# fateshelled/onnx_image_processing

Hardware: AMD Instinct MI355X
Metric: image-pairs/sec (640x480, K=512) (higher is better)
Workload: dtype f32; 1 GPU; Shi-Tomasi(3) + NMS(r=5)/top-k + sparse BAD(512, hard) + Sinkhorn(20, eps 0.05) + MNN(100, 0.1), 640x480 gray pairs, K=512 (BASELINE configs[1]); height=480, width=640, max_keypoints=512, parallelism=pair-sharded x1, input=float32 frames resident in HBM

## Files before the change

### onnx_image_processing_amd/csrc/hooks.h

```cpp
#pragma once

#ifdef MI_DEBUG_HOOKS
#include <atomic>
struct MiHooks {
  std::atomic<int> corner_impl{0};
  std::atomic<int> corner_rows{4};
  std::atomic<int> corner_rows_u8_default{1};
  std::atomic<int> sinkhorn_log_partials{0};
  std::atomic<int> sinkhorn_split{2};
  std::atomic<int> sinkhorn_persist{1};
  std::atomic<int> sinkhorn_stamps{0};
  std::atomic<int> topk_select{1};
  std::atomic<int> sinkhorn_schedule{-1};
  std::atomic<int> akaze_impl{0};
  std::atomic<int> bad_oriented_impl{0};
  std::atomic<int> cost_impl{0};
  std::atomic<int> sinkhorn_mix{1};
  std::atomic<int> sinkhorn_pair_waves{1};
  std::atomic<int> mnn_pair_waves{1};
  std::atomic<int> sinkhorn_exp_rows{1};
  std::atomic<int> mnn_one_pass{1};
  std::atomic<int> nms_impl{0};
  std::atomic<int> topk_split{-1};
  std::atomic<unsigned long long *> corner_clk{nullptr};
  std::atomic<unsigned long long *> topk_prof{nullptr};
};
extern MiHooks mi_hooks;
#define MI_HOOK(field, product_value) (mi_hooks.field.load(std::memory_order_relaxed))
#else
#define MI_HOOK(field, product_value) (product_value)
#endif
```

### onnx_image_processing_amd/csrc/hooks.hip

```cpp
#ifndef MI_DEBUG_HOOKS
#error "hooks.hip belongs to the debug library only (-DMI_DEBUG_HOOKS)"
#endif
#include "common.h"
#include "hooks.h"

#include "../../include/mi355x_match_debug.h"

MiHooks mi_hooks;

int mi_bad_plan_passes_host(const uint32_t *pair_geom_host, int num_pairs, int *canonical, int *scheduled);
int mi_sinkhorn_dots_form_host(int batch, int n, int m, int flags, int blocks_per_cu, int cus);

MI_API int mi_debug_clock_probe(void *buffer) {
  mi_hooks.corner_clk = reinterpret_cast<unsigned long long *>(buffer);
  return MI_OK;
}

MI_API int mi_debug_topk_stamps(void *buffer) {
  mi_hooks.topk_prof = reinterpret_cast<unsigned long long *>(buffer);
  return MI_OK;
}

MI_API int mi_debug_set(int key, int value) {
  if (key == 0) {
    mi_hooks.corner_impl = 0; mi_hooks.corner_rows = 4; mi_hooks.corner_rows_u8_default = 1;
    mi_hooks.sinkhorn_log_partials = 0; mi_hooks.sinkhorn_split = 2; mi_hooks.sinkhorn_persist = 1;
    mi_hooks.sinkhorn_stamps = 0; mi_hooks.topk_select = 1; mi_hooks.topk_split = -1; mi_hooks.sinkhorn_schedule = -1;
    mi_hooks.akaze_impl = 0;
    mi_hooks.bad_oriented_impl = 0;
    mi_hooks.cost_impl = 0;
    mi_hooks.sinkhorn_mix = 1;
    mi_hooks.sinkhorn_pair_waves = 1;
    mi_hooks.mnn_pair_waves = 1;
    mi_hooks.mnn_one_pass = 1;
    mi_hooks.sinkhorn_exp_rows = 1;
    mi_hooks.nms_impl = 0;
    mi_hooks.corner_clk = nullptr; mi_hooks.topk_prof = nullptr;
    return MI_OK;
  }
  if (key == 1) { mi_hooks.corner_impl = value; return MI_OK; }
  if (key == 2 && (value == 4 || value == 5 || value == 8)) { mi_hooks.corner_rows = value; mi_hooks.corner_rows_u8_default = 0; return MI_OK; }
  if (key == 4) { mi_hooks.sinkhorn_log_partials = value; return MI_OK; }
  if (key == 6) { mi_hooks.sinkhorn_split = value; return MI_OK; }
  if (key == 7) { mi_hooks.sinkhorn_persist = value; return MI_OK; }
  if (key == 8) { mi_hooks.sinkhorn_stamps = value; return MI_OK; }
  if (key == 9) { mi_hooks.topk_select = value; return MI_OK; }
  if (key == 10) { mi_hooks.topk_split = value; return MI_OK; }
  if (key == 12 && (value == 0 || value == 1)) { mi_hooks.akaze_impl = value; return MI_OK; }
  if (key == 13 && (value == 0 || value == 1)) { mi_hooks.bad_oriented_impl = value; return MI_OK; }
  if (key == 14 && (value == 0 || value == 1)) { mi_hooks.cost_impl = value; return MI_OK; }
  if (key == 15 && (value == 0 || value == 1)) { mi_hooks.sinkhorn_mix = value; return MI_OK; }
  if (key == 16 && (value == 0 || value == 1)) { mi_hooks.sinkhorn_pair_waves = value; return MI_OK; }
  if (key == 17 && (value == 0 || value == 1)) { mi_hooks.mnn_pair_waves = value; return MI_OK; }
  if (key == 19 && (value == 0 || value == 1)) { mi_hooks.mnn_one_pass = value; return MI_OK; }
  if (key == 18 && (value == 0 || value == 1)) { mi_hooks.sinkhorn_exp_rows = value; return MI_OK; }
  if (key == 20 && (value == 0 || value == 1)) { mi_hooks.nms_impl = value; return MI_OK; }
  if (key == 11 && value >= -1 && value <= 2) { mi_hooks.sinkhorn_schedule = value; return MI_OK; }
  return MI_E_PARAM;
}

MI_API int mi_debug_bad_plan_passes(const uint32_t *pair_geom_host, int num_pairs, int *canonical, int *scheduled) {
  return mi_bad_plan_passes_host(pair_geom_host, num_pairs, canonical, scheduled);
}

#include "sk_tuner.h"
MI_API int mi_debug_tuner_script(int n_ops, const int *op, const int *arg, const double *val, int *out) {
  if (n_ops < 0 || (n_ops > 0 && (!op || !arg || !val || !out))) return MI_E_NULL;
  mi::TunerLogic t;
  int last_entry = -1, last_slot = -1;
  for (int i = 0; i < n_ops; ++i) {
    mi::TunerShape s;
    s.batch = arg[i]; s.n = 512; s.m = 512; s.iterations = 20;
    switch (op[i]) {
      case 0: {
        const int sched = t.begin(s, &last_entry, &last_slot);
        out[i] = sched | ((last_slot & 0xff) << 8) | ((last_entry & 0xff) << 16);
        break;
      }
      case 1: t.finish(arg[i] >> 8, arg[i] & 0xff, val[i]); out[i] = 0; break;
      case 2: t.abandon(arg[i] >> 8, arg[i] & 0xff); out[i] = 0; break;
      case 3: out[i] = t.current(s); break;
      case 4: out[i] = t.for_capture(s); break;
      case 5: out[i] = t.set(arg[i]) ? 0 : -1; break;
      default: return MI_E_PARAM;
    }
  }
  return MI_OK;
}

MI_API int mi_debug_sinkhorn_dots_form(int batch, int n, int m, int flags, int blocks_per_cu, int cus) {
  return mi_sinkhorn_dots_form_host(batch, n, m, flags, blocks_per_cu, cus);
}

#include "akaze_math.h"
namespace {
__global__ __launch_bounds__(256) void akaze_math_check_kernel(int which, float kappa, uint32_t lo_bits, uint32_t hi_bits,
                                                               unsigned long long *mismatches, uint32_t *first_bad) {
  const float rk = 1.0f / kappa;
  unsigned long long bad = 0;
  for (unsigned long long b = (unsigned long long)lo_bits + blockIdx.x * 256ull + threadIdx.x; b < hi_bits;
       b += (unsigned long long)gridDim.x * 256ull) {
    const float x = __uint_as_float((uint32_t)b);
    float got, want;
    if (which == 0) { got = ak_sqrt(x); want = sqrtf(x); }
    else if (which == 1) { got = ak_div_by(x, kappa, rk); want = x / kappa; }
    else if (which == 2) { got = ak_rcp(x); want = 1.0f / x; }
    else if (which == 3) { got = ak_div(x, kappa); want = x / kappa; }
    else if (which == 4) { got = ak_sqrt_fp<1>(x); want = sqrtf(x); }
    else { got = ak_sqrt_fp<2>(x); want = sqrtf(x); }
    if (__float_as_uint(got) != __float_as_uint(want)) {
      ++bad;
      atomicMin(first_bad, (uint32_t)b);
    }
  }
  if (bad) atomicAdd(mismatches, bad);
}
}

MI_API int mi_debug_akaze_math_check(int which, float kappa, uint32_t lo_bits, uint32_t hi_bits, void *mismatches_u64,
                                     void *first_bad_u32, mi_stream_t stream) {
  MI_ENTER();
  if (!mismatches_u64 || !first_bad_u32) return MI_E_NULL;
  if (which < 0 || which > 5 || !(kappa > 0.0f) || lo_bits >= hi_bits) return MI_E_PARAM;
  hipLaunchKernelGGL(akaze_math_check_kernel, dim3(4096), dim3(256), 0, (hipStream_t)stream, which, kappa, lo_bits, hi_bits,
                     reinterpret_cast<unsigned long long *>(mismatches_u64), reinterpret_cast<uint32_t *>(first_bad_u32));
  return mi_launch_status();
}
```

### onnx_image_processing_amd/csrc/topk.hip

```cpp
#include "common.h"

#include "hooks.h"

namespace {

constexpr int TK_THREADS = 1024;
constexpr int TK_WAVES = TK_THREADS / 64;
constexpr int TK_MAX = 4096;
constexpr int TK_SEGS = 1024;

__device__ __forceinline__ void bitonic_sort_desc(uint64_t *keys, int npad, int t) {
  for (int size = 2; size <= npad; size <<= 1) {
    for (int stride = size >> 1; stride > 0; stride >>= 1) {
      for (int i = t; i < (npad >> 1); i += TK_THREADS) {
        const int pos = 2 * i - (i & (stride - 1));
        const int par = pos + stride;
        const bool desc = ((pos & size) == 0);
        const uint64_t a = keys[pos], b = keys[par];
        if ((a < b) == desc) {
          keys[pos] = b;
          keys[par] = a;
        }
      }
      __syncthreads();
    }
  }
}

template <int SIZE, int STRIDE>
__device__ __forceinline__ void bitonic_stage_4096(uint64_t (&r)[4], uint64_t *keys, uint64_t *keys2, int t, int &flip) {
  if constexpr (STRIDE < 4) {
#pragma unroll
    for (int j = 0; j < 4; ++j) {
      if ((j ^ STRIDE) > j) {
        const bool desc = (((t * 4 + j) & SIZE) == 0);
        const uint64_t a = r[j], b = r[j ^ STRIDE];
        const bool sw = (a < b) == desc;
        r[j] = sw ? b : a;
        r[j ^ STRIDE] = sw ? a : b;
      }
    }
  } else {
    uint64_t other[4];
    if constexpr (STRIDE < 256) {
#pragma unroll
      for (int j = 0; j < 4; ++j) other[j] = __shfl_xor(r[j], STRIDE >> 2, 64);
    } else {
      uint64_t *buf = flip ? keys2 : keys;
      flip ^= 1;
#pragma unroll
      for (int j = 0; j < 4; ++j) buf[t * 4 + j] = r[j];
      __syncthreads();
      const int pt = t ^ (STRIDE >> 2);
#pragma unroll
      for (int j = 0; j < 4; ++j) other[j] = buf[pt * 4 + j];
    }
    const bool lower = (t & (STRIDE >> 2)) == 0;
#pragma unroll
    for (int j = 0; j < 4; ++j) {
      const bool desc = (((t * 4 + j) & SIZE) == 0);
      const bool gt = r[j] > other[j];
      const uint64_t mx = gt ? r[j] : other[j], mn = gt ? other[j] : r[j];
      r[j] = (lower == desc) ? mx : mn;
    }
  }
}

template <int SIZE, int STRIDE>
__device__ __forceinline__ void bitonic_merge_4096(uint64_t (&r)[4], uint64_t *keys, uint64_t *keys2, int t, int &flip) {
  if constexpr (STRIDE >= 1) {
    bitonic_stage_4096<SIZE, STRIDE>(r, keys, keys2, t, flip);
    bitonic_merge_4096<SIZE, STRIDE / 2>(r, keys, keys2, t, flip);
  }
}

template <int SIZE>
__device__ __forceinline__ void bitonic_levels_4096(uint64_t (&r)[4], uint64_t *keys, uint64_t *keys2, int t, int &flip) {
  if constexpr (SIZE <= TK_MAX) {
    bitonic_merge_4096<SIZE, SIZE / 2>(r, keys, keys2, t, flip);
    bitonic_levels_4096<SIZE * 2>(r, keys, keys2, t, flip);
  }
}

__device__ __forceinline__ void bitonic_sort_desc_4096(uint64_t *keys, uint64_t *keys2, int t) {
  uint64_t r[4];
#pragma unroll
  for (int j = 0; j < 4; ++j) r[j] = keys[t * 4 + j];
  int flip = 0;
  bitonic_levels_4096<2>(r, keys, keys2, t, flip);
  __syncthreads();
#pragma unroll
  for (int j = 0; j < 4; ++j) keys[t * 4 + j] = r[j];
  __syncthreads();
}

constexpr int TK_BIG_MAX = 32768;

template <bool BIG>
__global__ __launch_bounds__(TK_THREADS) void topk_kernel(const uint64_t *__restrict__ cand,
                                                          const uint32_t *__restrict__ count, int segments,
                                                          uint32_t seg_cap, int w, int k, MiSets kpt_sets,
                                                          float *__restrict__ kscores, int select_mode,
                                                          unsigned long long *prof) {
#define TK_STAMP(i) do { if (prof && blockIdx.x == 0 && threadIdx.x == 0) prof[i] = wall_clock64(); } while (0)
  TK_STAMP(0);
  __shared__ uint64_t raw[BIG ? TK_BIG_MAX / 2 : 2 * TK_MAX];
  uint64_t *const keys = raw;
  uint64_t *const keys2 = raw + TK_MAX;
  uint32_t *const scores = reinterpret_cast<uint32_t *>(raw);
  __shared__ uint32_t seg_cnt[TK_SEGS], seg_base[TK_SEGS];
  __shared__ uint32_t hist[256];
  __shared__ uint32_t wsum[TK_WAVES];
  __shared__ uint64_t s_prefix;
  __shared__ uint32_t s_krem, s_fill, s_done;

  const int t = threadIdx.x, lane = t & 63, wave = t >> 6;
  const int img = blockIdx.x;
  const uint64_t *list = cand + (size_t)img * segments * seg_cap;
  const uint32_t *cnt = count + (size_t)img * segments;

  const bool slots = segments <= TK_SEGS;
  uint32_t part = 0;
  if (t == 0) s_fill = 0u;
  __syncthreads();
  for (int s = t; s < segments; s += TK_THREADS) {
    const uint32_t c = min(cnt[s], seg_cap);
    part += c;
    if (slots) {
      seg_cnt[s] = c;
      seg_base[s] = c ? atomicAdd(&s_fill, c) : 0u;
    }
  }
#pragma unroll
  for (int o = 32; o > 0; o >>= 1) part += __shfl_xor(part, o, 64);
  if (lane == 0) wsum[wave] = part;
  __syncthreads();
  uint32_t n = 0;
#pragma unroll
  for (int q = 0; q < TK_WAVES; ++q) n += wsum[q];
  int nsel;
  TK_STAMP(1);

  bool in_lds = false;
  if (BIG && slots && n > (uint32_t)TK_MAX && n <= (uint32_t)TK_BIG_MAX && k <= TK_MAX) {
    for (int s0 = wave * 8; s0 < segments; s0 += TK_WAVES * 8) {
      uint64_t v[8];
      uint32_t c[8], base[8];
#pragma unroll
      for (int q = 0; q < 8; ++q) {
        const int sg = s0 + q;
        c[q] = sg < segments ? seg_cnt[sg] : 0u;
        base[q] = sg < segments ? seg_base[sg] : 0u;
        v[q] = 0ull;
        if ((uint32_t)lane < c[q]) v[q] = list[(size_t)sg * seg_cap + lane];
      }
#pragma unroll
      for (int q = 0; q < 8; ++q) {
        if ((uint32_t)lane < c[q]) scores[base[q] + lane] = (uint32_t)(v[q] >> 32);
        for (uint32_t i = 64 + lane; i < c[q]; i += 64) scores[base[q] + i] = (uint32_t)(list[(size_t)(s0 + q) * seg_cap + i] >> 32);
      }
    }
    if (t == 0) { s_prefix = 0ull; s_krem = (uint32_t)k; s_done = 0u; }
    __syncthreads();
    uint32_t mask32 = 0u;
    for (int shift = 24; shift >= 0; shift -= 8) {
      if (t < 256) hist[t] = 0u;
      __syncthreads();
      const uint32_t prefix = (uint32_t)s_prefix;
      for (uint32_t i0 = 0; i0 < n; i0 += TK_THREADS) {
        const uint32_t i = i0 + t;
        const uint32_t sc = i < n ? scores[i] : 0u;
        const bool act = i < n && ((sc & mask32) == prefix);
        const uint32_t digit = (sc >> shift) & 255u;
        const unsigned long long am = __ballot(act);
        if (am) {
          const int leader = __ffsll((long long)am) - 1;
          const uint32_t d0 = __shfl(digit, leader, 64);
          const unsigned long long same = __ballot(act && digit == d0);
          if (lane == leader) atomicAdd(&hist[d0], (uint32_t)__popcll(same));
          if (act && digit != d0) atomicAdd(&hist[digit], 1u);
        }
      }
      __syncthreads();
      if (t < 64) {
        const uint32_t krem = s_krem;
        uint32_t c[4], tot = 0;
#pragma unroll
        for (int q = 0; q < 4; ++q) { c[q] = hist[255 - 4 * t - q]; tot += c[q]; }
        uint32_t incl = tot;
#pragma unroll
        for (int o = 1; o < 64; o <<= 1) {
          const uint32_t up = __shfl_up(incl, o, 64);
          if (t >= o) incl += up;
        }
        uint32_t above = incl - tot;
        if (above < krem && krem <= incl) {
#pragma unroll
          for (int q = 0; q < 4; ++q) {
            if (krem <= above + c[q]) {
              s_prefix = (uint64_t)(prefix | ((uint32_t)(255 - 4 * t - q) << shift));
              s_krem = krem - above;
              s_fill = c[q];
              if (krem - above == c[q]) s_done = 1u;
              break;
            }
            above += c[q];
          }
        }
      }
      mask32 |= (0xFFu << shift);
      __syncthreads();
      if (s_done) break;
    }
    const uint32_t floor32 = (uint32_t)s_prefix;
    const uint32_t n2 = ((uint32_t)k - s_krem) + s_fill;
    __syncthreads();
    if (n2 <= (uint32_t)TK_MAX) {
      if (t == 0) s_fill = 0u;
      __syncthreads();
      for (int s0 = wave * 8; s0 < segments; s0 += TK_WAVES * 8) {
        uint64_t v[8];
        uint32_t c[8];
#pragma unroll
        for (int q = 0; q < 8; ++q) {
          const int sg = s0 + q;
          c[q] = sg < segments ? seg_cnt[sg] : 0u;
          v[q] = 0ull;
          if ((uint32_t)lane < c[q]) v[q] = list[(size_t)sg * seg_cap + lane];
        }
#pragma unroll
        for (int q = 0; q < 8; ++q) {
          if ((uint32_t)lane < c[q] && (uint32_t)(v[q] >> 32) >= floor32) keys[atomicAdd(&s_fill, 1u)] = v[q];
          for (uint32_t i = 64 + lane; i < c[q]; i += 64) {
            const uint64_t key = list[(size_t)(s0 + q) * seg_cap + i];
            if ((uint32_t)(key >> 32) >= floor32) keys[atomicAdd(&s_fill, 1u)] = key;
          }
        }
      }
      __syncthreads();
      n = s_fill;
      in_lds = true;
    }
    __syncthreads();
  }

  if (in_lds || (n <= (uint32_t)TK_MAX && slots)) {
    for (int s0 = wave * 4; !in_lds && s0 < segments; s0 += TK_WAVES * 4) {
      uint64_t v[4];
      uint32_t c[4], base[4];
#pragma unroll
      for (int q = 0; q < 4; ++q) {
        const int sg = s0 + q;
        c[q] = sg < segments ? seg_cnt[sg] : 0u;
        base[q] = sg < segments ? seg_base[sg] : 0u;
        v[q] = 0ull;
        if ((uint32_t)lane < c[q]) v[q] = list[(size_t)sg * seg_cap + lane];
      }
#pragma unroll
      for (int q = 0; q < 4; ++q) {
        if ((uint32_t)lane < c[q]) keys[base[q] + lane] = v[q];
        for (uint32_t i = 64 + lane; i < c[q]; i += 64) keys[base[q] + i] = list[(size_t)(s0 + q) * seg_cap + i];
      }
    }
    int npad = 2;
    while (npad < (int)n) npad <<= 1;
    __syncthreads();
    TK_STAMP(2);
    if ((select_mode || in_lds) && n >= (uint32_t)k && 4 * k <= TK_MAX && (n > (uint32_t)k || in_lds)) {
      uint64_t r[4];
#pragma unroll
      for (int q = 0; q < 4; ++q) r[q] = (uint32_t)(t + q * TK_THREADS) < n ? keys[t + q * TK_THREADS] : 0ull;
      if (t == 0) { s_prefix = 0ull; s_krem = (uint32_t)k; s_fill = 0u; s_done = 0u; }
      uint64_t mask = 0ull;
      for (int shift = n == (uint32_t)k ? -8 : 56; shift >= 0; shift -= 8) {
        if (t < 256) hist[t] = 0u;
        __syncthreads();
        const uint64_t prefix = s_prefix;
#pragma unroll
        for (int q = 0; q < 4; ++q) {
          const bool act = r[q] != 0ull && ((r[q] & mask) == prefix);
          const uint32_t digit = (uint32_t)(r[q] >> shift) & 255u;
          const unsigned long long am = __ballot(act);
          if (am) {
            const int leader = __ffsll((long long)am) - 1;
            const uint32_t d0 = __shfl(digit, leader, 64);
            const unsigned long long same = __ballot(act && digit == d0);
            if (lane == leader) atomicAdd(&hist[d0], (uint32_t)__popcll(same));
            if (act && digit != d0) atomicAdd(&hist[digit], 1u);
          }
        }
        __syncthreads();
        if (t < 64) {
          const uint32_t krem = s_krem;
          uint32_t c[4], tot = 0;
#pragma unroll
          for (int q = 0; q < 4; ++q) { c[q] = hist[255 - 4 * t - q]; tot += c[q]; }
          uint32_t incl = tot;
#pragma unroll
          for (int o = 1; o < 64; o <<= 1) {
            const uint32_t up = __shfl_up(incl, o, 64);
            if (t >= o) incl += up;
          }
          uint32_t above = incl - tot;
          if (above < krem && krem <= incl) {
#pragma unroll
            for (int q = 0; q < 4; ++q) {
              if (krem <= above + c[q]) {
                s_prefix = prefix | ((uint64_t)(255 - 4 * t - q) << shift);
                s_krem = krem - above;
                if (krem - above == c[q]) s_done = 1u;
                break;
              }
              above += c[q];
            }
          }
        }
        mask |= (0xFFull << shift);
        __syncthreads();
        if (s_done) break;
      }
      if (n == (uint32_t)k) __syncthreads();
      const uint64_t kth = s_prefix;
      TK_STAMP(3);
#pragma unroll
      for (int q = 0; q < 4; ++q)
        if (r[q] != 0ull && r[q] >= kth) {
          const uint32_t slot = atomicAdd(&s_fill, 1u);
          if (slot < (uint32_t)TK_MAX) keys2[slot] = r[q];
        }
      __syncthreads();
      nsel = (int)(s_fill < (uint32_t)k ? s_fill : (uint32_t)k);
      int kpad = 2;
      while (kpad < k) kpad <<= 1;
      for (int i = nsel + t; i < kpad; i += TK_THREADS) keys2[i] = 0ull;
      __syncthreads();
      TK_STAMP(4);
      if (kpad >= 128 && kpad <= TK_THREADS) {
        const int tpk = TK_THREADS / kpad, slice = kpad / tpk;
        const int ki = t & (kpad - 1), part = t / kpad;
        if (t < kpad) seg_cnt[t] = 0u;
        const uint64_t mine = keys2[ki];
        uint32_t above = 0;
        if (mine != 0ull) {
          const ulonglong2 *lst = reinterpret_cast<const ulonglong2 *>(keys2 + part * slice);
#pragma unroll 8
          for (int j = 0; j < slice / 2; ++j) {
            const ulonglong2 two = lst[j];
            above += (two.x > mine ? 1u : 0u) + (two.y > mine ? 1u : 0u);
          }
        }
        __syncthreads();
        if (mine != 0ull && above) atomicAdd(&seg_cnt[ki], above);
        __syncthreads();
        if (part == 0 && mine != 0ull) keys[seg_cnt[ki]] = mine;
        __syncthreads();
      } else {
        bitonic_sort_desc(keys2, kpad, t);
        for (int i = t; i < nsel; i += TK_THREADS) keys[i] = keys2[i];
        __syncthreads();
      }
    } else {
    for (int i = (int)n + t; i < npad; i += TK_THREADS) keys[i] = 0ull;
    __syncthreads();
    if (npad == TK_MAX) bitonic_sort_desc_4096(keys, keys2, t);
    else bitonic_sort_desc(keys, npad, t);
    nsel = (int)n < k ? (int)n : k;
    }
  } else if (n <= (uint32_t)TK_MAX) {
    for (int s = wave; s < segments; s += TK_WAVES) {
      const uint32_t c = min(cnt[s], seg_cap);
      if (c == 0u) continue;
      uint32_t base = 0;
      if (lane == 0) base = atomicAdd(&s_fill, c);
      base = __shfl(base, 0, 64);
      const uint64_t *seg = list + (size_t)s * seg_cap;
      for (uint32_t i = lane; i < c; i += 64) keys[base + i] = seg[i];
    }
    int npad = 2;
    while (npad < (int)n) npad <<= 1;
    __syncthreads();
    for (int i = (int)n + t; i < npad; i += TK_THREADS) keys[i] = 0ull;
    __syncthreads();
    if (npad == TK_MAX) bitonic_sort_desc_4096(keys, keys2, t);
    else bitonic_sort_desc(keys, npad, t);
    nsel = (int)n < k ? (int)n : k;
  } else {
    if (t == 0) { s_prefix = 0ull; s_krem = (uint32_t)k; s_fill = 0u; s_done = 0u; }
    uint64_t mask = 0ull;
    for (int shift = 56; shift >= 0; shift -= 8) {
      if (t < 256) hist[t] = 0u;
      __syncthreads();
      const uint64_t prefix = s_prefix;
      for (int s = wave; s < segments; s += TK_WAVES) {
        const uint32_t c = min(cnt[s], seg_cap);
        const uint64_t *seg = list + (size_t)s * seg_cap;
        for (uint32_t base = 0; base < c; base += 64) {
          const uint32_t i = base + lane;
          bool act = false;
          uint32_t digit = 0;
          if (i < c) {
            const uint64_t key = seg[i];
            act = ((key & mask) == prefix);
            digit = (uint32_t)(key >> shift) & 255u;
          }
          const unsigned long long am = __ballot(act);
          if (am) {
            const int leader = __ffsll((long long)am) - 1;
            const uint32_t d0 = __shfl(digit, leader, 64);
            const unsigned long long same = __ballot(act && digit == d0);
            if (lane == leader) atomicAdd(&hist[d0], (uint32_t)__popcll(same));
            if (act && digit != d0) atomicAdd(&hist[digit], 1u);
          }
        }
      }
      __syncthreads();
      if (t < 64) {
        const uint32_t krem = s_krem;
        uint32_t c[4], tot = 0;
#pragma unroll
        for (int q = 0; q < 4; ++q) { c[q] = hist[255 - 4 * t - q]; tot += c[q]; }
        uint32_t incl = tot;
#pragma unroll
        for (int o = 1; o < 64; o <<= 1) {
          const uint32_t v = __shfl_up(incl, o, 64);
          if (t >= o) incl += v;
        }
        uint32_t above = incl - tot;
        if (above < krem && krem <= incl) {
#pragma unroll
          for (int q = 0; q < 4; ++q) {
            if (krem <= above + c[q]) {
              s_prefix = prefix | ((uint64_t)(255 - 4 * t - q) << shift);
              s_krem = krem - above;
              if (krem - above == c[q]) s_done = 1u;
              break;
            }
            above += c[q];
          }
        }
      }
      mask |= (0xFFull << shift);
      __syncthreads();
      if (s_done) break;
    }
    const uint64_t kth = s_prefix;
    for (int s = wave; s < segments; s += TK_WAVES) {
      const uint32_t c = min(cnt[s], seg_cap);
      const uint64_t *seg = list + (size_t)s * seg_cap;
      for (uint32_t i = lane; i < c; i += 64) {
        const uint64_t key = seg[i];
        if (key >= kth) {
          const uint32_t slot = atomicAdd(&s_fill, 1u);
          if (slot < (uint32_t)TK_MAX) keys[slot] = key;
        }
      }
    }
    __syncthreads();
    nsel = (int)(s_fill < (uint32_t)k ? s_fill : (uint32_t)k);
    int npad = 2;
    while (npad < k) npad <<= 1;
    for (int i = nsel + t; i < npad; i += TK_THREADS) keys[i] = 0ull;
    __syncthreads();
    bitonic_sort_desc(keys, npad, t);
  }

  TK_STAMP(5);
  float *kpts = const_cast<float *>(mi_set_item<float>(kpt_sets, img, (size_t)k * 2));
  for (int j = t; j < k; j += TK_THREADS) {
    float y = -1.0f, x = -1.0f, s = 0.0f;
    if (j < nsel) {
      const uint64_t key = keys[j];
      const uint32_t lin = 0xFFFFFFFFu - (uint32_t)(key & 0xFFFFFFFFull);
      y = (float)(lin / (uint32_t)w);
      x = (float)(lin % (uint32_t)w);
      s = __uint_as_float((uint32_t)(key >> 32));
    }
    kpts[(size_t)j * 2 + 0] = y;
    kpts[(size_t)j * 2 + 1] = x;
    kscores[(size_t)img * k + j] = s;
  }
  TK_STAMP(6);
#undef TK_STAMP
}

}

int mi_topk_keypoints_sets(const uint64_t *cand, const uint32_t *count, int segments, int segment_capacity, int n, int w,
                           int k, MiSets keypoints, float *kscores, mi_stream_t stream) {
  if (!cand || !count || !keypoints.a || (keypoints.per_set < n && !keypoints.b) || !kscores) return MI_E_NULL;
  if (n <= 0 || w <= 0 || segments <= 0) return MI_E_SHAPE;
  if (k <= 0 || k > TK_MAX) return MI_E_PARAM;
  if (segment_capacity <= 0) return MI_E_CAPACITY;
  const int choice = MI_HOOK(topk_split, -1);
  const bool big = choice < 0 ? segments > 150 : choice != 0;
  if (big)
    hipLaunchKernelGGL(topk_kernel<true>, dim3(n), dim3(TK_THREADS), 0, (hipStream_t)stream, cand, count, segments,
                       (uint32_t)segment_capacity, w, k, keypoints, kscores, MI_HOOK(topk_select, 1),
                       MI_HOOK(topk_prof, (unsigned long long *)nullptr));
  else
    hipLaunchKernelGGL(topk_kernel<false>, dim3(n), dim3(TK_THREADS), 0, (hipStream_t)stream, cand, count, segments,
                       (uint32_t)segment_capacity, w, k, keypoints, kscores, MI_HOOK(topk_select, 1),
                       MI_HOOK(topk_prof, (unsigned long long *)nullptr));
  return mi_launch_status();
}

extern "C" int mi_topk_keypoints(const uint64_t *cand, const uint32_t *count, int segments,
                                 int segment_capacity, int n, int w, int k, float *keypoints, float *kscores,
                                 mi_stream_t stream) {
  MI_ENTER();
  return mi_topk_keypoints_sets(cand, count, segments, segment_capacity, n, w, k, mi_one_set(keypoints, n), kscores, stream);
}
```

Measured before the change: 219,000 image-pairs/sec.

## Rework top-k kernel: 512-thread form, direct segment prefetch, wider radix select, register bitonic sort

Templates the top-k kernel on workgroup size and by default launches a 512-thread variant for the small-segment path with K≤1024. When there are few segments it prefetches candidate keys into registers and computes segment bases with a DPP wave scan instead of shared atomics. Radix select moves from 8-bit to 11/10-bit digits with double-buffered histograms, and winner compaction uses ballot/mbcnt. The final sort becomes a register-resident bitonic sort using DPP lane exchanges. This cuts LDS traffic, barriers and select passes, and the smaller block should allow higher occupancy. In exchange it adds considerable code complexity and a risk of correctness bugs.

```diff
diff --git a/onnx_image_processing_amd/csrc/hooks.h b/onnx_image_processing_amd/csrc/hooks.h
--- a/onnx_image_processing_amd/csrc/hooks.h
+++ b/onnx_image_processing_amd/csrc/hooks.h
@@ -22,6 +22,7 @@
   std::atomic<int> mnn_one_pass{1};
   std::atomic<int> nms_impl{0};
   std::atomic<int> topk_split{-1};
+  std::atomic<int> topk_form{-1};
   std::atomic<unsigned long long *> corner_clk{nullptr};
   std::atomic<unsigned long long *> topk_prof{nullptr};
 };
diff --git a/onnx_image_processing_amd/csrc/hooks.hip b/onnx_image_processing_amd/csrc/hooks.hip
--- a/onnx_image_processing_amd/csrc/hooks.hip
+++ b/onnx_image_processing_amd/csrc/hooks.hip
@@ -35,6 +35,7 @@
     mi_hooks.mnn_one_pass = 1;
     mi_hooks.sinkhorn_exp_rows = 1;
     mi_hooks.nms_impl = 0;
+    mi_hooks.topk_form = -1;
     mi_hooks.corner_clk = nullptr; mi_hooks.topk_prof = nullptr;
     return MI_OK;
   }
@@ -55,6 +56,7 @@
   if (key == 19 && (value == 0 || value == 1)) { mi_hooks.mnn_one_pass = value; return MI_OK; }
   if (key == 18 && (value == 0 || value == 1)) { mi_hooks.sinkhorn_exp_rows = value; return MI_OK; }
   if (key == 20 && (value == 0 || value == 1)) { mi_hooks.nms_impl = value; return MI_OK; }
+  if (key == 21 && (value == -1 || value == 512 || value == 1024)) { mi_hooks.topk_form = value; return MI_OK; }
   if (key == 11 && value >= -1 && value <= 2) { mi_hooks.sinkhorn_schedule = value; return MI_OK; }
   return MI_E_PARAM;
 }
diff --git a/onnx_image_processing_amd/csrc/topk.hip b/onnx_image_processing_amd/csrc/topk.hip
--- a/onnx_image_processing_amd/csrc/topk.hip
+++ b/onnx_image_processing_amd/csrc/topk.hip
@@ -4,15 +4,44 @@
 
 namespace {
 
-constexpr int TK_THREADS = 1024;
-constexpr int TK_WAVES = TK_THREADS / 64;
 constexpr int TK_MAX = 4096;
 constexpr int TK_SEGS = 1024;
-
+constexpr int TK_SEGS_SMALL = 256;
+constexpr int TK_BINS = 2048;
+
+template <int CTRL>
+__device__ __forceinline__ uint64_t dpp_u64(uint64_t v) {
+  const int lo = (int)(uint32_t)v, hi = (int)(uint32_t)(v >> 32);
+  const uint32_t l = (uint32_t)__builtin_amdgcn_update_dpp(lo, lo, CTRL, 0xf, 0xf, false);
+  const uint32_t h = (uint32_t)__builtin_amdgcn_update_dpp(hi, hi, CTRL, 0xf, 0xf, false);
+  return ((uint64_t)h << 32) | l;
+}
+
+template <int X>
+__device__ __forceinline__ uint64_t lane_xor_u64(uint64_t v) {
+  if constexpr (X == 1) return dpp_u64<0xB1>(v);
+  else if constexpr (X == 2) return dpp_u64<0x4E>(v);
+  else if constexpr (X == 4) return dpp_u64<0x1B>(dpp_u64<0x141>(v));
+  else if constexpr (X == 8) return dpp_u64<0x128>(v);
+  else return __shfl_xor(v, X, 64);
+}
+
+__device__ __forceinline__ uint32_t wave_scan_dpp(uint32_t x) {
+  int v = (int)x;
+  v += __builtin_amdgcn_update_dpp(0, v, 0x111, 0xf, 0xf, false);
+  v += __builtin_amdgcn_update_dpp(0, v, 0x112, 0xf, 0xf, false);
+  v += __builtin_amdgcn_update_dpp(0, v, 0x114, 0xf, 0xf, false);
+  v += __builtin_amdgcn_update_dpp(0, v, 0x118, 0xf, 0xf, false);
+  v += __builtin_amdgcn_update_dpp(0, v, 0x142, 0xa, 0xf, false);
+  v += __builtin_amdgcn_update_dpp(0, v, 0x143, 0xc, 0xf, false);
+  return (uint32_t)v;
+}
+
+template <int WGT>
 __device__ __forceinline__ void bitonic_sort_desc(uint64_t *keys, int npad, int t) {
   for (int size = 2; size <= npad; size <<= 1) {
     for (int stride = size >> 1; stride > 0; stride >>= 1) {
-      for (int i = t; i < (npad >> 1); i += TK_THREADS) {
+      for (int i = t; i < (npad >> 1); i += WGT) {
         const int pos = 2 * i - (i & (stride - 1));
         const int par = pos + stride;
         const bool desc = ((pos & size) == 0);
@@ -27,13 +56,14 @@
   }
 }
 
-template <int SIZE, int STRIDE>
-__device__ __forceinline__ void bitonic_stage_4096(uint64_t (&r)[4], uint64_t *keys, uint64_t *keys2, int t, int &flip) {
-  if constexpr (STRIDE < 4) {
-#pragma unroll
-    for (int j = 0; j < 4; ++j) {
+template <int N, int KPT, bool PING, int WGT, int SIZE, int STRIDE>
+__device__ __forceinline__ void bitonic_stage_reg(uint64_t (&r)[KPT], uint64_t *buf, int t, bool active, int &flip) {
+  constexpr int NT = N / KPT;
+  if constexpr (STRIDE < KPT) {
+#pragma unroll
+    for (int j = 0; j < KPT; ++j) {
       if ((j ^ STRIDE) > j) {
-        const bool desc = (((t * 4 + j) & SIZE) == 0);
+        const bool desc = (((t * KPT + j) & SIZE) == 0);
         const uint64_t a = r[j], b = r[j ^ STRIDE];
         const bool sw = (a < b) == desc;
         r[j] = sw ? b : a;
@@ -41,24 +71,33 @@
       }
     }
   } else {
-    uint64_t other[4];
-    if constexpr (STRIDE < 256) {
-#pragma unroll
-      for (int j = 0; j < 4; ++j) other[j] = __shfl_xor(r[j], STRIDE >> 2, 64);
+    uint64_t other[KPT];
+#pragma unroll
+    for (int j = 0; j < KPT; ++j) other[j] = 0ull;
+    if constexpr (STRIDE < 64 * KPT) {
+      if (active) {
+#pragma unroll
+        for (int j = 0; j < KPT; ++j) other[j] = lane_xor_u64<STRIDE / KPT>(r[j]);
+      }
     } else {
-      uint64_t *buf = flip ? keys2 : keys;
+      uint64_t *b = buf + ((PING && flip) ? N : 0);
       flip ^= 1;
-#pragma unroll
-      for (int j = 0; j < 4; ++j) buf[t * 4 + j] = r[j];
-      __syncthreads();
-      const int pt = t ^ (STRIDE >> 2);
-#pragma unroll
-      for (int j = 0; j < 4; ++j) other[j] = buf[pt * 4 + j];
-    }
-    const bool lower = (t & (STRIDE >> 2)) == 0;
-#pragma unroll
-    for (int j = 0; j < 4; ++j) {
-      const bool desc = (((t * 4 + j) & SIZE) == 0);
+      if (active) {
+#pragma unroll
+        for (int j = 0; j < KPT; ++j) b[j * NT + t] = r[j];
+      }
+      __syncthreads();
+      const int pt = t ^ (STRIDE / KPT);
+      if (active) {
+#pragma unroll
+        for (int j = 0; j < KPT; ++j) other[j] = b[j * NT + pt];
+      }
+      if constexpr (!PING) __syncthreads();
+    }
+    const bool lower = (t & (STRIDE / KPT)) == 0;
+#pragma unroll
+    for (int j = 0; j < KPT; ++j) {
+      const bool desc = (((t * KPT + j) & SIZE) == 0);
       const bool gt = r[j] > other[j];
       const uint64_t mx = gt ? r[j] : other[j], mn = gt ? other[j] : r[j];
       r[j] = (lower == desc) ? mx : mn;
@@ -66,50 +105,61 @@
   }
 }
 
-template <int SIZE, int STRIDE>
-__device__ __forceinline__ void bitonic_merge_4096(uint64_t (&r)[4], uint64_t *keys, uint64_t *keys2, int t, int &flip) {
+template <int N, int KPT, bool PING, int WGT, int SIZE, int STRIDE>
+__device__ __forceinline__ void bitonic_merge_reg(uint64_t (&r)[KPT], uint64_t *buf, int t, bool active, int &flip) {
   if constexpr (STRIDE >= 1) {
-    bitonic_stage_4096<SIZE, STRIDE>(r, keys, keys2, t, flip);
-    bitonic_merge_4096<SIZE, STRIDE / 2>(r, keys, keys2, t, flip);
-  }
-}
-
-template <int SIZE>
-__device__ __forceinline__ void bitonic_levels_4096(uint64_t (&r)[4], uint64_t *keys, uint64_t *keys2, int t, int &flip) {
-  if constexpr (SIZE <= TK_MAX) {
-    bitonic_merge_4096<SIZE, SIZE / 2>(r, keys, keys2, t, flip);
-    bitonic_levels_4096<SIZE * 2>(r, keys, keys2, t, flip);
-  }
-}
-
-__device__ __forceinline__ void bitonic_sort_desc_4096(uint64_t *keys, uint64_t *keys2, int t) {
-  uint64_t r[4];
-#pragma unroll
-  for (int j = 0; j < 4; ++j) r[j] = keys[t * 4 + j];
+    bitonic_stage_reg<N, KPT, PING, WGT, SIZE, STRIDE>(r, buf, t, active, flip);
+    bitonic_merge_reg<N, KPT, PING, WGT, SIZE, STRIDE / 2>(r, buf, t, active, flip);
+  }
+}
+
+template <int N, int KPT, bool PING, int WGT, int SIZE>
+__device__ __forceinline__ void bitonic_levels_reg(uint64_t (&r)[KPT], uint64_t *buf, int t, bool active, int &flip) {
+  if constexpr (SIZE <= N) {
+    bitonic_merge_reg<N, KPT, PING, WGT, SIZE, SIZE / 2>(r, buf, t, active, flip);
+    bitonic_levels_reg<N, KPT, PING, WGT, SIZE * 2>(r, buf, t, active, flip);
+  }
+}
+
+template <int N, int KPT, bool PING, int WGT>
+__device__ __forceinline__ void bitonic_sort_desc_reg(uint64_t *keys, int t, int nvalid) {
+  static_assert(N % (64 * KPT) == 0 && N / KPT <= WGT, "whole waves own the keys");
+  asm volatile("" : "+v"(t));
+  const bool active = (N / KPT == WGT) || t < N / KPT;
+  uint64_t r[KPT];
+#pragma unroll
+  for (int j = 0; j < KPT; ++j) r[j] = (active && t * KPT + j < nvalid) ? keys[t * KPT + j] : 0ull;
+  __syncthreads();
   int flip = 0;
-  bitonic_levels_4096<2>(r, keys, keys2, t, flip);
+  bitonic_levels_reg<N, KPT, PING, WGT, 2>(r, keys, t, active, flip);
   __syncthreads();
-#pragma unroll
-  for (int j = 0; j < 4; ++j) keys[t * 4 + j] = r[j];
+  if (active) {
+#pragma unroll
+    for (int j = 0; j < KPT; ++j) keys[t * KPT + j] = r[j];
+  }
   __syncthreads();
 }
 
 constexpr int TK_BIG_MAX = 32768;
 
-template <bool BIG>
-__global__ __launch_bounds__(TK_THREADS) void topk_kernel(const uint64_t *__restrict__ cand,
-                                                          const uint32_t *__restrict__ count, int segments,
-                                                          uint32_t seg_cap, int w, int k, MiSets kpt_sets,
-                                                          float *__restrict__ kscores, int select_mode,
-                                                          unsigned long long *prof) {
+template <bool BIG, int WGT>
+__global__ __launch_bounds__(WGT, BIG ? 4 : 8) void topk_kernel(const uint64_t *__restrict__ cand,
+                                                                const uint32_t *__restrict__ count, int segments,
+                                                                uint32_t seg_cap, int w, int k, MiSets kpt_sets,
+                                                                float *__restrict__ kscores, int select_mode,
+                                                                unsigned long long *prof) {
 #define TK_STAMP(i) do { if (prof && blockIdx.x == 0 && threadIdx.x == 0) prof[i] = wall_clock64(); } while (0)
   TK_STAMP(0);
-  __shared__ uint64_t raw[BIG ? TK_BIG_MAX / 2 : 2 * TK_MAX];
+  constexpr int TK_THREADS = WGT, TK_WAVES = WGT / 64;
+  constexpr int KPT = TK_MAX / WGT;
+  constexpr int SEGS = BIG ? TK_SEGS : TK_SEGS_SMALL;
+  constexpr bool REG_SORT_ALL = WGT == 1024;
+  __shared__ __align__(16) uint64_t raw[BIG ? TK_BIG_MAX / 2 : TK_MAX];
   uint64_t *const keys = raw;
-  uint64_t *const keys2 = raw + TK_MAX;
   uint32_t *const scores = reinterpret_cast<uint32_t *>(raw);
-  __shared__ uint32_t seg_cnt[TK_SEGS], seg_base[TK_SEGS];
-  __shared__ uint32_t hist[256];
+  __shared__ uint32_t seg_cnt[SEGS], seg_base[SEGS];
+  __shared__ __align__(16) uint32_t hist_own[BIG ? 2 * TK_BINS : 4];
+  uint32_t *const hist = BIG ? hist_own : reinterpret_cast<uint32_t *>(raw);
   __shared__ uint32_t wsum[TK_WAVES];
   __shared__ uint64_t s_prefix;
   __shared__ uint32_t s_krem, s_fill, s_done;
@@ -119,22 +169,43 @@
   const uint64_t *list = cand + (size_t)img * segments * seg_cap;
   const uint32_t *cnt = count + (size_t)img * segments;
 
-  const bool slots = segments <= TK_SEGS;
+  const bool slots = segments <= SEGS;
+  constexpr int PRE = BIG ? 1 : 80 / TK_WAVES;
+  const bool direct = !BIG && segments <= PRE * TK_WAVES;
+  uint64_t pre[PRE];
+  uint32_t my_cnt = 0u, my_base = 0u;
   uint32_t part = 0;
   if (t == 0) s_fill = 0u;
-  __syncthreads();
-  for (int s = t; s < segments; s += TK_THREADS) {
-    const uint32_t c = min(cnt[s], seg_cap);
-    part += c;
-    if (slots) {
-      seg_cnt[s] = c;
-      seg_base[s] = c ? atomicAdd(&s_fill, c) : 0u;
-    }
-  }
-#pragma unroll
-  for (int o = 32; o > 0; o >>= 1) part += __shfl_xor(part, o, 64);
+  if (direct) {
+    const int mine = wave + lane * TK_WAVES;
+    const uint32_t raw_cnt = cnt[min(mine, segments - 1)];
+#pragma unroll
+    for (int q = 0; q < PRE; ++q) {
+      const int sg = min(wave + q * TK_WAVES, segments - 1);
+      pre[q] = list[(size_t)sg * seg_cap + min((uint32_t)lane, seg_cap - 1u)];
+    }
+    if (lane < PRE && mine < segments) my_cnt = min(raw_cnt, seg_cap);
+    const uint32_t incl = wave_scan_dpp(my_cnt);
+    my_base = incl - my_cnt;
+    part = (uint32_t)__builtin_amdgcn_readlane((int)incl, 63);
+  } else {
+    __syncthreads();
+    for (int s = t; s < segments; s += TK_THREADS) {
+      const uint32_t c = min(cnt[s], seg_cap);
+      part += c;
+      if (slots) {
+        seg_cnt[s] = c;
+        seg_base[s] = c ? atomicAdd(&s_fill, c) : 0u;
+      }
+    }
+#pragma unroll
+    for (int o = 32; o > 0; o >>= 1) part += __shfl_xor(part, o, 64);
+  }
   if (lane == 0) wsum[wave] = part;
   __syncthreads();
+  uint32_t wave_base = 0;
+#pragma unroll
+  for (int q = 0; q < TK_WAVES; ++q) wave_base += q < wave ? wsum[q] : 0u;
   uint32_t n = 0;
 #pragma unroll
   for (int q = 0; q < TK_WAVES; ++q) n += wsum[q];
@@ -245,7 +316,24 @@
   }
 
   if (in_lds || (n <= (uint32_t)TK_MAX && slots)) {
-    for (int s0 = wave * 4; !in_lds && s0 < segments; s0 += TK_WAVES * 4) {
+    if (direct) {
+#pragma unroll
+      for (int q = 0; q < PRE; ++q) {
+        const uint32_t c = (uint32_t)__builtin_amdgcn_readlane((int)my_cnt, q);
+        const uint32_t base = wave_base + (uint32_t)__builtin_amdgcn_readlane((int)my_base, q);
+        if ((uint32_t)lane < c) keys[base + lane] = pre[q];
+      }
+      unsigned long long longer = __ballot(my_cnt > 64u);
+      while (longer) {
+        const int q = __ffsll((long long)longer) - 1;
+        longer &= longer - 1ull;
+        const uint32_t c = (uint32_t)__builtin_amdgcn_readlane((int)my_cnt, q);
+        const uint32_t base = wave_base + (uint32_t)__builtin_amdgcn_readlane((int)my_base, q);
+        const uint64_t *seg = list + (size_t)(wave + q * TK_WAVES) * seg_cap;
+        for (uint32_t i = 64 + lane; i < c; i += 64) keys[base + i] = seg[i];
+      }
+    }
+    for (int s0 = wave * 4; !in_lds && !direct && s0 < segments; s0 += TK_WAVES * 4) {
       uint64_t v[4];
       uint32_t c[4], base[4];
 #pragma unroll
@@ -267,103 +355,102 @@
     __syncthreads();
     TK_STAMP(2);
     if ((select_mode || in_lds) && n >= (uint32_t)k && 4 * k <= TK_MAX && (n > (uint32_t)k || in_lds)) {
-      uint64_t r[4];
-#pragma unroll
-      for (int q = 0; q < 4; ++q) r[q] = (uint32_t)(t + q * TK_THREADS) < n ? keys[t + q * TK_THREADS] : 0ull;
+      uint64_t r[KPT];
       if (t == 0) { s_prefix = 0ull; s_krem = (uint32_t)k; s_fill = 0u; s_done = 0u; }
+#pragma unroll
+      for (int q = 0; q < KPT; ++q) r[q] = (uint32_t)(t + q * TK_THREADS) < n ? keys[t + q * TK_THREADS] : 0ull;
+      __syncthreads();
       uint64_t mask = 0ull;
-      for (int shift = n == (uint32_t)k ? -8 : 56; shift >= 0; shift -= 8) {
-        if (t < 256) hist[t] = 0u;
+      int shift = 64;
+      if (n != (uint32_t)k) {
+        for (uint32_t i = t; i < (uint32_t)TK_BINS; i += TK_THREADS) hist[i] = 0u;
         __syncthreads();
+      }
+      for (int p = 0; p < 6 && n != (uint32_t)k; ++p) {
+        const int bits = (p % 3 == 2) ? 10 : 11;
+        const uint32_t nb = 1u << bits;
+        shift -= bits;
+        uint32_t *const h = hist + (p & 1) * TK_BINS, *const hnext = hist + ((p & 1) ^ 1) * TK_BINS;
         const uint64_t prefix = s_prefix;
 #pragma unroll
-        for (int q = 0; q < 4; ++q) {
+        for (int q = 0; q < KPT; ++q) {
           const bool act = r[q] != 0ull && ((r[q] & mask) == prefix);
-          const uint32_t digit = (uint32_t)(r[q] >> shift) & 255u;
+          const uint32_t digit = (uint32_t)(r[q] >> shift) & (nb - 1u);
           const unsigned long long am = __ballot(act);
           if (am) {
             const int leader = __ffsll((long long)am) - 1;
-            const uint32_t d0 = __shfl(digit, leader, 64);
+            const uint32_t d0 = (uint32_t)__builtin_amdgcn_readlane((int)digit, leader);
             const unsigned long long same = __ballot(act && digit == d0);
-            if (lane == leader) atomicAdd(&hist[d0], (uint32_t)__popcll(same));
-            if (act && digit != d0) atomicAdd(&hist[digit], 1u);
-          }
-        }
+            if (act && (digit != d0 || lane == leader)) atomicAdd(&h[digit], lane == leader ? (uint32_t)__popcll(same) : 1u);
+          }
+        }
+        for (uint32_t i = t; i < (uint32_t)TK_BINS; i += TK_THREADS) hnext[i] = 0u;
         __syncthreads();
         if (t < 64) {
           const uint32_t krem = s_krem;
-          uint32_t c[4], tot = 0;
-#pragma unroll
-          for (int q = 0; q < 4; ++q) { c[q] = hist[255 - 4 * t - q]; tot += c[q]; }
-          uint32_t incl = tot;
-#pragma unroll
-          for (int o = 1; o < 64; o <<= 1) {
-            const uint32_t up = __shfl_up(incl, o, 64);
-            if (t >= o) incl += up;
-          }
-          uint32_t above = incl - tot;
-          if (above < krem && krem <= incl) {
-#pragma unroll
-            for (int q = 0; q < 4; ++q) {
-              if (krem <= above + c[q]) {
-                s_prefix = prefix | ((uint64_t)(255 - 4 * t - q) << shift);
-                s_krem = krem - above;
-                if (krem - above == c[q]) s_done = 1u;
-                break;
-              }
-              above += c[q];
+          const uint32_t per = nb >> 6;
+          const uint4 *blk = reinterpret_cast<const uint4 *>(h + (nb - per * (uint32_t)(t + 1)));
+          uint32_t tot = 0;
+          for (uint32_t i = 0; i < (per >> 2); ++i) {
+            const uint4 v = blk[(i + (uint32_t)t) & ((per >> 2) - 1u)];
+            tot += v.x + v.y + v.z + v.w;
+          }
+          const uint32_t incl = wave_scan_dpp(tot);
+          const uint32_t above = incl - tot;
+          const unsigned long long owner = __ballot(above < krem && krem <= incl);
+          if (owner) {
+            const int L = __ffsll((long long)owner) - 1;
+            const uint32_t above_l = (uint32_t)__builtin_amdgcn_readlane((int)above, L);
+            const uint32_t bin = nb - 1u - per * (uint32_t)L - (uint32_t)t;
+            const uint32_t c = (uint32_t)t < per ? h[bin] : 0u;
+            const uint32_t ab2 = above_l + wave_scan_dpp(c) - c;
+            if ((uint32_t)t < per && ab2 < krem && krem <= ab2 + c) {
+              s_prefix = prefix | ((uint64_t)bin << shift);
+              s_krem = krem - ab2;
+              if (krem - ab2 == c) s_done = 1u;
             }
           }
         }
-        mask |= (0xFFull << shift);
+        mask |= ((uint64_t)(nb - 1u) << shift);
         __syncthreads();
         if (s_done) break;
       }
-      if (n == (uint32_t)k) __syncthreads();
       const uint64_t kth = s_prefix;
       TK_STAMP(3);
-#pragma unroll
-      for (int q = 0; q < 4; ++q)
-        if (r[q] != 0ull && r[q] >= kth) {
-          const uint32_t slot = atomicAdd(&s_fill, 1u);
-          if (slot < (uint32_t)TK_MAX) keys2[slot] = r[q];
-        }
+      unsigned long long wm[KPT];
+      uint32_t wins = 0;
+#pragma unroll
+      for (int q = 0; q < KPT; ++q) {
+        wm[q] = __ballot(r[q] != 0ull && r[q] >= kth);
+        wins += (uint32_t)__popcll(wm[q]);
+      }
+      uint32_t base = 0u;
+      if (lane == 0 && wins) base = atomicAdd(&s_fill, wins);
+      base = (uint32_t)__builtin_amdgcn_readfirstlane((int)base);
+#pragma unroll
+      for (int q = 0; q < KPT; ++q) {
+        const uint32_t slot = base + __builtin_amdgcn_mbcnt_hi((uint32_t)(wm[q] >> 32), __builtin_amdgcn_mbcnt_lo((uint32_t)wm[q], 0u));
+        if (r[q] != 0ull && r[q] >= kth && slot < (uint32_t)TK_MAX) keys[slot] = r[q];
+        base += (uint32_t)__popcll(wm[q]);
+      }
       __syncthreads();
       nsel = (int)(s_fill < (uint32_t)k ? s_fill : (uint32_t)k);
-      int kpad = 2;
-      while (kpad < k) kpad <<= 1;
-      for (int i = nsel + t; i < kpad; i += TK_THREADS) keys2[i] = 0ull;
-      __syncthreads();
       TK_STAMP(4);
-      if (kpad >= 128 && kpad <= TK_THREADS) {
-        const int tpk = TK_THREADS / kpad, slice = kpad / tpk;
-        const int ki = t & (kpad - 1), part = t / kpad;
-        if (t < kpad) seg_cnt[t] = 0u;
-        const uint64_t mine = keys2[ki];
-        uint32_t above = 0;
-        if (mine != 0ull) {
-          const ulonglong2 *lst = reinterpret_cast<const ulonglong2 *>(keys2 + part * slice);
-#pragma unroll 8
-          for (int j = 0; j < slice / 2; ++j) {
-            const ulonglong2 two = lst[j];
-            above += (two.x > mine ? 1u : 0u) + (two.y > mine ? 1u : 0u);
-          }
-        }
-        __syncthreads();
-        if (mine != 0ull && above) atomicAdd(&seg_cnt[ki], above);
-        __syncthreads();
-        if (part == 0 && mine != 0ull) keys[seg_cnt[ki]] = mine;
-        __syncthreads();
-      } else {
-        bitonic_sort_desc(keys2, kpad, t);
-        for (int i = t; i < nsel; i += TK_THREADS) keys[i] = keys2[i];
-        __syncthreads();
-      }
+      if (k <= 512) bitonic_sort_desc_reg<512, 1, true, WGT>(keys, t, nsel);
+      else bitonic_sort_desc_reg<1024, (WGT < 1024 ? 1024 / WGT : 1), true, WGT>(keys, t, nsel);
     } else {
-    for (int i = (int)n + t; i < npad; i += TK_THREADS) keys[i] = 0ull;
-    __syncthreads();
-    if (npad == TK_MAX) bitonic_sort_desc_4096(keys, keys2, t);
-    else bitonic_sort_desc(keys, npad, t);
+    bool sorted = false;
+    if constexpr (REG_SORT_ALL) {
+      if (npad == TK_MAX) {
+        bitonic_sort_desc_reg<TK_MAX, KPT, BIG, WGT>(keys, t, (int)n);
+        sorted = true;
+      }
+    }
+    if (!sorted) {
+      for (int i = (int)n + t; i < npad; i += TK_THREADS) keys[i] = 0ull;
+      __syncthreads();
+      bitonic_sort_desc<WGT>(keys, npad, t);
+    }
     nsel = (int)n < k ? (int)n : k;
     }
   } else if (n <= (uint32_t)TK_MAX) {
@@ -381,8 +468,14 @@
     __syncthreads();
     for (int i = (int)n + t; i < npad; i += TK_THREADS) keys[i] = 0ull;
     __syncthreads();
-    if (npad == TK_MAX) bitonic_sort_desc_4096(keys, keys2, t);
-    else bitonic_sort_desc(keys, npad, t);
+    bool sorted = false;
+    if constexpr (REG_SORT_ALL) {
+      if (npad == TK_MAX) {
+        bitonic_sort_desc_reg<TK_MAX, KPT, BIG, WGT>(keys, t, npad);
+        sorted = true;
+      }
+    }
+    if (!sorted) bitonic_sort_desc<WGT>(keys, npad, t);
     nsel = (int)n < k ? (int)n : k;
   } else {
     if (t == 0) { s_prefix = 0ull; s_krem = (uint32_t)k; s_fill = 0u; s_done = 0u; }
@@ -461,7 +554,7 @@
     while (npad < k) npad <<= 1;
     for (int i = nsel + t; i < npad; i += TK_THREADS) keys[i] = 0ull;
     __syncthreads();
-    bitonic_sort_desc(keys, npad, t);
+    bitonic_sort_desc<WGT>(keys, npad, t);
   }
 
   TK_STAMP(5);
@@ -493,14 +586,19 @@
   if (segment_capacity <= 0) return MI_E_CAPACITY;
   const int choice = MI_HOOK(topk_split, -1);
   const bool big = choice < 0 ? segments > 150 : choice != 0;
+  const int forced = MI_HOOK(topk_form, -1);
+  const int form = forced > 0 ? forced : k > 1024 ? 1024 : 512;
+  const int select = MI_HOOK(topk_select, 1);
+  unsigned long long *const prof = MI_HOOK(topk_prof, (unsigned long long *)nullptr);
   if (big)
-    hipLaunchKernelGGL(topk_kernel<true>, dim3(n), dim3(TK_THREADS), 0, (hipStream_t)stream, cand, count, segments,
-                       (uint32_t)segment_capacity, w, k, keypoints, kscores, MI_HOOK(topk_select, 1),
-                       MI_HOOK(topk_prof, (unsigned long long *)nullptr));
+    hipLaunchKernelGGL((topk_kernel<true, 1024>), dim3(n), dim3(1024), 0, (hipStream_t)stream, cand, count, segments,
+                       (uint32_t)segment_capacity, w, k, keypoints, kscores, select, prof);
+  else if (form == 1024)
+    hipLaunchKernelGGL((topk_kernel<false, 1024>), dim3(n), dim3(1024), 0, (hipStream_t)stream, cand, count, segments,
+                       (uint32_t)segment_capacity, w, k, keypoints, kscores, select, prof);
   else
-    hipLaunchKernelGGL(topk_kernel<false>, dim3(n), dim3(TK_THREADS), 0, (hipStream_t)stream, cand, count, segments,
-                       (uint32_t)segment_capacity, w, k, keypoints, kscores, MI_HOOK(topk_select, 1),
-                       MI_HOOK(topk_prof, (unsigned long long *)nullptr));
+    hipLaunchKernelGGL((topk_kernel<false, 512>), dim3(n), dim3(512), 0, (hipStream_t)stream, cand, count, segments,
+                       (uint32_t)segment_capacity, w, k, keypoints, kscores, select, prof);
   return mi_launch_status();
 }
 
```

Result: no change. 221,100 image-pairs/sec, median of 6 (+1.0%).
